# jwliao1209/DiffMusic

Hardware: AMD Instinct MI355X
Metric: denoising steps/sec (10 s clip, 200-step DPS) (higher is better)
Workload: dtype f16; 1 GPU; MusicLDM + DPS music_inpainting, 10 s @16 kHz, 200-step schedule, batch 8 per GPU (BASELINE.json configs[1]); global_batch=8, clips_per_gpu=8, lanes=1, parallelism=clip-sharded x1 (RCCL world size 1, no per-step collective), finite=True, nan_steps=0, settle_steps=10, cached_reference_transform=True, launched_by=single process

## Files before the change

diffmusic_amd/_lib.py:

```python
import ctypes as C
import os

_HERE = os.path.dirname(os.path.abspath(__file__))
LIB_PATH = os.environ.get("DMX_LIB_PATH") or os.path.join(_HERE, "lib", "libdiffmusic_hip.so")
MAX_STAGES = 8


class HifiGanConfig(C.Structure):
    _fields_ = [("model_in_dim", C.c_int), ("upsample_initial_channel", C.c_int), ("num_upsamples", C.c_int),
                ("upsample_rates", C.c_int * MAX_STAGES), ("upsample_kernel_sizes", C.c_int * MAX_STAGES),
                ("num_kernels", C.c_int), ("resblock_kernel_sizes", C.c_int * MAX_STAGES),
                ("num_dilations", C.c_int), ("resblock_dilation_sizes", C.c_int * (MAX_STAGES * MAX_STAGES)),
                ("leaky_relu_slope", C.c_float)]


class VaeConfig(C.Structure):
    _fields_ = [("latent_channels", C.c_int), ("out_channels", C.c_int), ("num_blocks", C.c_int),
                ("block_out_channels", C.c_int * MAX_STAGES), ("layers_per_block", C.c_int),
                ("norm_num_groups", C.c_int), ("eps", C.c_float)]


class UNetConfig(C.Structure):
    _fields_ = [("in_channels", C.c_int), ("out_channels", C.c_int), ("num_blocks", C.c_int),
                ("block_out_channels", C.c_int * MAX_STAGES), ("layers_per_block", C.c_int),
# ... 69 lines not shown
    "dmx_unet_workspace_bytes": (C.c_size_t, [C.c_void_p, C.c_int, C.c_int, C.c_int]),
    "dmx_unet_fwd": (C.c_int, [C.c_void_p, C.c_void_p, C.c_void_p, C.c_void_p, C.c_void_p, C.c_int, C.c_int, C.c_int,
                               C.c_void_p, C.c_size_t, C.c_void_p]),
    "dmx_unet_fwd_ctx": (C.c_int, [C.c_void_p] * 5 + [C.c_int, C.c_void_p, C.c_int, C.c_void_p, C.c_void_p, C.c_int, C.c_int, C.c_int,
                                   C.c_void_p, C.c_size_t, C.c_void_p]),
    "dmx_unet_workspace_bytes_ctx": (C.c_size_t, [C.c_void_p, C.c_int, C.c_int, C.c_int, C.c_int, C.c_int]),
    "dmx_htsat_create": (C.c_void_p, [C.POINTER(HtsatConfig)]),
    "dmx_htsat_feature_dims": (C.c_int, [C.c_void_p, C.POINTER(C.c_int), C.POINTER(C.c_int)]),
    "dmx_htsat_workspace_bytes": (C.c_size_t, [C.c_void_p, C.c_int, C.c_int]),
    "dmx_htsat_fwd": (C.c_int, [C.c_void_p, C.c_void_p, C.c_int, C.c_int, C.c_void_p, C.c_int, C.c_void_p, C.c_size_t, C.c_void_p]),
    "dmx_htsat_bwd": (C.c_int, [C.c_void_p, C.c_void_p, C.c_void_p, C.c_void_p, C.c_void_p]),
    "dmx_htsat_tape_raw": (C.c_size_t, [C.c_void_p, C.c_int, C.c_int, C.c_int, C.c_void_p, C.c_size_t, C.c_void_p]),
    "dmx_gram_fwd": (C.c_int, [C.c_void_p, C.c_void_p, C.c_int, C.c_int, C.c_int, C.c_void_p]),
    "dmx_gram_bwd": (C.c_int, [C.c_void_p, C.c_void_p, C.c_void_p, C.c_int, C.c_int, C.c_int, C.c_void_p]),
    "dmx_gemm_raw": (C.c_int, [C.c_void_p, C.c_size_t, C.c_void_p]),
    "dmx_prof_begin": (None, []),
    "dmx_prof_end": (C.c_int, [C.POINTER(C.c_double), C.POINTER(C.c_double)]),
    "dmx_flash_attn_raw": (C.c_int, [C.c_void_p, C.c_void_p, C.c_void_p, C.c_void_p, C.c_void_p] + [C.c_int] * 6 + [C.c_float, C.c_void_p]),
    "dmx_flash_attn_ld_raw": (C.c_int, [C.c_void_p] * 5 + [C.c_int] * 8 + [C.c_float, C.POINTER(C.c_int), C.c_void_p]),
    "dmx_softmax_raw": (C.c_int, [C.c_void_p] * 3 + [C.c_longlong, C.c_int, C.c_longlong, C.c_longlong, C.c_int, C.c_void_p]),
    "dmx_softmax_act_raw": (C.c_int, [C.c_void_p] * 3 + [C.c_longlong, C.c_int, C.c_longlong, C.c_int, C.c_void_p]),
    "dmx_transpose_raw": (C.c_int, [C.c_void_p, C.c_void_p, C.c_int, C.c_int, C.c_longlong, C.c_longlong, C.c_int, C.c_int] + [C.c_longlong] * 4
                          + [C.c_void_p]),
    "dmx_rowdot_raw": (C.c_int, [C.c_void_p] * 3 + [C.c_longlong, C.c_int, C.c_longlong, C.c_longlong, C.c_void_p]),
    "dmx_layernorm_raw": (C.c_int, [C.c_void_p] * 4 + [C.c_int, C.c_int, C.c_float, C.c_void_p]),
    "dmx_geglu_raw": (C.c_int, [C.c_void_p, C.c_void_p, C.c_longlong, C.c_int, C.c_void_p]),
    "dmx_gemm_splitk_workspace": (C.c_int, [C.c_void_p, C.c_size_t]),
    "dmx_conv_pair_raw": (C.c_int, [C.c_void_p, C.c_void_p, C.c_size_t, C.c_void_p]),
    "dmx_conv_pair_group_raw": (C.c_int, [C.c_int, C.c_void_p, C.c_void_p, C.c_size_t, C.c_void_p]),
    "dmx_conv_pair_dead_raw": (C.c_int, [C.c_void_p, C.c_void_p, C.c_size_t, C.POINTER(C.c_int), C.POINTER(C.c_int), C.POINTER(C.c_int), C.c_void_p]),
# ... 150 lines not shown
```

diffmusic_amd/csrc/capi.hip:

```cpp
#include "conv_pair.h"
#include "models.h"

#define M_IMPL(m) ((m) ? (m)->impl : nullptr)
#define ST(s) ((hipStream_t)(s))

extern "C" {

int dmx_abi_version(void) { return DMX_ABI_VERSION; }
int dmx_act_dtype(void) { return DMX_ACT_DTYPE; }

dmx_model* dmx_hifigan_create(const dmx_hifigan_config* cfg) {
  if (!cfg || cfg->num_upsamples > DMX_MAX_STAGES || cfg->num_kernels > DMX_MAX_STAGES || cfg->num_dilations > DMX_MAX_STAGES) {
    dmx_set_error("bad hifigan config");
    return nullptr;
  }
  return new dmx_model{dmx_make_hifigan(cfg)};
}
dmx_model* dmx_vae_decoder_create(const dmx_vae_config* cfg) {
  if (!cfg || cfg->num_blocks > DMX_MAX_STAGES) { dmx_set_error("bad vae config"); return nullptr; }
  Model* m = dmx_make_vae(cfg);
  return m ? new dmx_model{m} : nullptr;
}
dmx_model* dmx_unet_create(const dmx_unet_config* cfg) {
  if (!cfg || cfg->num_blocks > DMX_MAX_STAGES) { dmx_set_error("bad unet config"); return nullptr; }
// ... 143 lines not shown
                 void* ws, size_t ws_bytes, void* stream) {
  int rc = check(m, DMX_MODEL_UNET);
  if (rc) return rc;
  if (!ws) { dmx_set_error("null workspace"); return DMX_ERR_WORKSPACE; }
  return dmx_unet_fwd_impl(m->impl, x, t, class_labels, eps, batch, h, w, ws, ws_bytes, ST(stream), nullptr, 0, nullptr, 0, nullptr);
}
int dmx_unet_fwd_ctx(dmx_model* m, const float* x, const float* t, const float* class_labels, const float* ctx0, int n0,
                     const float* ctx1, int n1, const float* bias1, float* eps, int batch, int h, int w, void* ws, size_t ws_bytes,
                     void* stream) {
  int rc = check(m, DMX_MODEL_UNET);
  if (rc) return rc;
  if (!ws) { dmx_set_error("null workspace"); return DMX_ERR_WORKSPACE; }
  return dmx_unet_fwd_impl(m->impl, x, t, class_labels, eps, batch, h, w, ws, ws_bytes, ST(stream), ctx0, n0, ctx1, n1, bias1);
}

static thread_local int g_raw_gn_rows = 0;
int dmx_gemm_raw(const void* desc, size_t desc_bytes, void* stream) {
  if (desc_bytes != sizeof(GemmDesc)) { dmx_set_error("GemmDesc size mismatch: %zu vs %zu", desc_bytes, sizeof(GemmDesc)); return DMX_ERR_SHAPE; }
  return dmx_gemm_launch(*reinterpret_cast<const GemmDesc*>(desc), ST(stream), &g_raw_gn_rows);
}
int dmx_gemm_last_tile_rows_raw(void) { return g_raw_gn_rows; }

int dmx_conv_pair_raw(const void* desc_a, const void* desc_b, size_t desc_bytes, void* stream) {
  if (desc_bytes != sizeof(GemmDesc)) { dmx_set_error("GemmDesc size mismatch: %zu vs %zu", desc_bytes, sizeof(GemmDesc)); return DMX_ERR_SHAPE; }
  const GemmDesc* a = reinterpret_cast<const GemmDesc*>(desc_a);
  const GemmDesc& b = *reinterpret_cast<const GemmDesc*>(desc_b);
  if (!dmx_conv_pair_eligible(a, b)) { dmx_set_error("shape not handled by the fused convolution-pair kernel"); return DMX_ERR_SHAPE; }
  return dmx_conv_pair_launch(a, b, ST(stream));
}

// ... 149 lines not shown
```

diffmusic_amd/csrc/dmx_common.h:

```cpp
#pragma once
#include <hip/hip_runtime.h>
#include <stdint.h>
#include <stddef.h>

typedef uint16_t act_t;

#define DMX_OK 0
#define DMX_ERR_SHAPE (-1)
#define DMX_ERR_WORKSPACE (-2)
#define DMX_ERR_PARAM (-3)
#define DMX_ERR_STATE (-4)
#define DMX_ERR_LAUNCH (-5)

typedef __attribute__((ext_vector_type(4))) float f32x4;
#ifdef DMX_BF16
typedef __bf16 native16_t;
typedef __attribute__((ext_vector_type(8))) __bf16 frag8_t;
#define DMX_MFMA16(a, b, c) __builtin_amdgcn_mfma_f32_16x16x32_bf16(a, b, c, 0, 0, 0)
#define DMX_ACT_DTYPE 0
#else
typedef _Float16 native16_t;
typedef __attribute__((ext_vector_type(8))) _Float16 frag8_t;
#define DMX_MFMA16(a, b, c) __builtin_amdgcn_mfma_f32_16x16x32_f16(a, b, c, 0, 0, 0)
#define DMX_ACT_DTYPE 1
// ... 108 lines not shown
  const act_t* gnb_x;
  const float* gnb_scale;
  const float* gnb_shift;
  int gnb_ldx, gnb_silu;
  const float* gnb_stats;
  int gnb_cpg;
};

int dmx_gemm_launch(const GemmDesc& d, hipStream_t stream, int* gn_rows = nullptr);
void dmx_gemm_set_splitk_workspace(float* ws, size_t bytes);
void dmx_gemm_release_splitk_workspace(const float* ws);
int dmx_gemm_launch_ln(int cfg, const GemmDesc& d, hipStream_t stream);
int dmx_gemm_launch_rowstats(int cfg, const GemmDesc& d, hipStream_t stream);
int dmx_gemm_launch_gnstats(int cfg, const GemmDesc& d, hipStream_t stream, int* gn_rows);
bool dmx_prof_is_active();
```

diffmusic_amd/csrc/gemm_conv.hip:

```cpp
#include "gemm_tile.h"

namespace {
template <int BM, int BN, int WM, int WN, int NSTAGE>
int launch_glds(const GemmDesc& d, hipStream_t stream) {
  if (d.flags & EPI_SOFTBWD) {
    if constexpr (BM == 256 && BN == 256) return launch_glds_t<BM, BN, WM, WN, NSTAGE, 2>(d, stream);
    else return DMX_ERR_SHAPE;
  }
  if (d.flags & EPI_GEGLU) return launch_glds_t<BM, BN, WM, WN, NSTAGE, 3>(d, stream);
  return (d.flags & (EPI_MASKBITS | EPI_BITS2)) ? launch_glds_t<BM, BN, WM, WN, NSTAGE, 1>(d, stream)
                                                : launch_glds_t<BM, BN, WM, WN, NSTAGE, 0>(d, stream);
}

template <int BM, int BN, int WM, int WN>
int launch_cfg(const GemmDesc& d, hipStream_t stream) {
  if (d.flags & EPI_SOFTBWD) return DMX_ERR_SHAPE;
  if (d.flags & EPI_GEGLU) {
    if constexpr ((BN / WN) % 32 == 0) return launch_cfg_t<BM, BN, WM, WN, 3>(d, stream);
    else return DMX_ERR_SHAPE;
  }
  return (d.flags & (EPI_MASKBITS | EPI_BITS2)) ? launch_cfg_t<BM, BN, WM, WN, 1>(d, stream) : launch_cfg_t<BM, BN, WM, WN, 0>(d, stream);
}

}

#include <vector>
// ... 5 lines not shown
int g_last_cfg = 0;
bool g_prof = false;
std::vector<ProfRec> g_prof_recs;
struct TileEntry { int M, N, K, Z, cfg; };
static const TileEntry g_tile_table[] = {
#include "tile_table.inc"
    {0, 0, 0, 0, 0}};

bool glds_ok(const GemmDesc& d) {
  const long long imgs = d.Hq * d.Wq > 0 ? (d.M + (long long)d.Hq * d.Wq - 1) / ((long long)d.Hq * d.Wq) : 1;
  const long long in_elems = (d.Hi > 1 || d.ntaps > 1 ? imgs * d.Hi * d.Wi : (long long)d.M) * d.lda;
  static const bool strided_ok = getenv("DMX_NO_GLDS_STRIDED") == nullptr;
  return in_elems < (1ll << 29) && (long long)d.M * d.lda < (1ll << 29) && ((long long)d.N + 512) * d.ldw < (1ll << 29) &&
         (d.sy == 1 || strided_ok);
}
int launch_by_cfg(int cfg, const GemmDesc& d, hipStream_t stream, int* gn_rows = nullptr) {
  g_last_cfg = cfg;
  if (d.flags & EPI_LNFOLD) return dmx_gemm_launch_ln(cfg, d, stream);
  if (d.flags & EPI_ROWSTATS) return dmx_gemm_launch_rowstats(cfg, d, stream);
  if (d.flags & (EPI_GNSTATS | EPI_GNBWD)) return dmx_gemm_launch_gnstats(cfg, d, stream, gn_rows);
  switch (cfg) {
    case 1: return launch_glds<256, 256, 2, 4, 2>(d, stream);
    case 2: return launch_glds<256, 128, 4, 2, 3>(d, stream);
    case 7: return launch_glds<320, 256, 2, 4, 2>(d, stream);
    case 8: return launch_glds<192, 256, 2, 4, 2>(d, stream);
    case 9: return launch_glds<320, 128, 4, 2, 2>(d, stream);
    case 10: return launch_glds<192, 128, 4, 2, 3>(d, stream);
    case 11: return launch_glds<128, 128, 2, 2, 2>(d, stream);
    case 12: return launch_glds<64, 64, 2, 2, 4>(d, stream);
    case 13: return launch_glds<128, 64, 2, 2, 3>(d, stream);
    case 14: return launch_glds<64, 128, 2, 2, 3>(d, stream);
    case 15: return launch_glds<64, 64, 2, 2, 8>(d, stream);
    case 16: return launch_glds<64, 128, 2, 2, 6>(d, stream);
    case 17: return launch_glds<128, 64, 2, 2, 6>(d, stream);
    case 18: return launch_glds<128, 128, 2, 2, 4>(d, stream);
    case 19: return launch_glds<512, 128, 4, 2, 2>(d, stream);
    case 3: return launch_cfg<128, 128, 2, 2>(d, stream);
    case 4: return launch_cfg<128, 64, 2, 2>(d, stream);
    case 5: return launch_cfg<128, 32, 4, 1>(d, stream);
    default: return launch_cfg<64, 64, 2, 2>(d, stream);
  }
}
int launch_dispatch(const GemmDesc& d, hipStream_t stream, int* gn_rows) {
  const bool gl = glds_ok(d);
  if (d.flags & EPI_SOFTBWD) return gl ? launch_by_cfg(1, d, stream, gn_rows) : DMX_ERR_SHAPE;
  if (d.tile_cfg >= 1 && d.tile_cfg <= 19 && ((d.tile_cfg > 2 && d.tile_cfg < 7) || gl)) return launch_by_cfg(d.tile_cfg, d, stream, gn_rows);
  {
    static int ovN[8], ovC[8], nov = -1;
    if (nov < 0) {
      nov = 0;
      if (const char* e = getenv("DMX_CFG_OVERRIDE")) {
        while (*e && nov < 8) {
          int n = 0, c = 0;
          if (sscanf(e, "%d:%d", &n, &c) == 2) { ovN[nov] = n; ovC[nov] = c; ++nov; }
          while (*e && *e != ',') ++e;
          if (*e == ',') ++e;
        }
      }
    }
    if (gl && d.M >= 40000)
      for (int i = 0; i < nov; ++i) if (ovN[i] == d.N) return launch_by_cfg(ovC[i], d, stream, gn_rows);
  }
  for (const TileEntry* e = g_tile_table; e->cfg; ++e)
    if (e->M == d.M && e->N == d.N && e->K == d.K && e->Z == d.Z) {
      const int c = e->cfg % 100;
      if ((c > 2 && c < 7) || gl) return launch_by_cfg(c, d, stream, gn_rows);
    }
  if (gl && d.M >= 2048 && d.N % 128 == 0) {
    auto cost = [&](int bm, int bn, int slots, double eff) {
      const double blocks = (double)cdiv(d.M, bm) * cdiv(d.N, bn) * d.Z;
      const double rounds = ceil(blocks / slots);
      return rounds * (bm / 128.0) * (bn / 128.0) * (slots / 256.0) / eff;
    };
    struct Cand { int cfg, bm, bn, slots; double eff; };
    static const Cand cands[] = {{1, 256, 256, 256, 0.95}, {7, 320, 256, 256, 0.93}, {8, 192, 256, 256, 0.88},
                                 {2, 256, 128, 256, 0.70}, {9, 320, 128, 256, 0.70}, {10, 192, 128, 256, 0.66},
                                 {19, 512, 128, 256, 0.75},
                                 {3, 128, 128, 512, 0.66}};
    int best = 0;
    double bc = 1e30;
    for (const Cand& c : cands) {
      if (c.bn == 256 && d.N % 256) continue;
      const double v = cost(c.bm, c.bn, c.slots, c.eff);
      if (v < bc) { bc = v; best = c.cfg; }
    }
    if (best && best != 3) return launch_by_cfg(best, d, stream, gn_rows);
  }
  if (d.N > 32 && (long long)cdiv(d.M, 128) * cdiv(d.N, 128) * d.Z < 200) {
    if (gl && d.K >= 512 && d.Z == 1) return launch_by_cfg(d.N % 128 == 0 && d.M >= 4000 ? 14 : 12, d, stream, gn_rows);
    return launch_by_cfg(6, d, stream, gn_rows);
  }
  if (d.N > 64) return launch_by_cfg(3, d, stream, gn_rows);
  if (d.N > 32) return launch_by_cfg(4, d, stream, gn_rows);
  return launch_by_cfg(5, d, stream, gn_rows);
}
}

bool dmx_prof_is_active() { return g_prof; }

extern "C" void dmx_prof_begin(void) {
// ... 14 lines not shown
  if (flops) *flops = g_dma_fl;
  if (bytes) *bytes = g_dma_by;
  return g_dma_n;
}
extern "C" int dmx_prof_end(double* total_ms, double* total_flops) {
  g_prof = false;
  g_dma_ms = g_dma_fl = g_dma_by = 0.0; g_dma_n = 0;
  (void)hipDeviceSynchronize();
  double ms = 0.0, fl = 0.0;
  FILE* csv = getenv("DMX_PROF_CSV") ? fopen(getenv("DMX_PROF_CSV"), "w") : nullptr;
  if (csv) fprintf(csv, "M,N,K,Z,taps,flags,cfg,ms,tflops\n");
  for (auto& r : g_prof_recs) {
    float t = 0.f;
    if (hipEventElapsedTime(&t, r.a, r.b) == hipSuccess) ms += t;
    if (csv) fprintf(csv, "%d,%d,%d,%d,%d,%d,%d,%.4f,%.1f\n", r.M, r.N, r.K, r.Z, r.taps, r.flags, r.cfg, t, t > 0 ? r.flops / t / 1e9 : 0.0);
    const bool dma = r.cfg == 1 || r.cfg == 2 || (r.cfg >= 7 && r.cfg <= 10) || r.cfg == 19;
    if (dma) { g_dma_ms += t; g_dma_fl += r.flops; g_dma_by += r.bytes; ++g_dma_n; }
    fl += r.flops;
    (void)hipEventDestroy(r.a); (void)hipEventDestroy(r.b);
  }
  if (csv) fclose(csv);
  const int n = (int)g_prof_recs.size();
  g_prof_recs.clear();
  if (total_ms) *total_ms = ms;
  if (total_flops) *total_flops = fl;
  return n;
}

namespace {
float* g_splitk_ws = nullptr;
size_t g_splitk_bytes = 0;
// ... 184 lines not shown
```

diffmusic_amd/csrc/gemm_tile.h:

```cpp
#pragma once
#include "dmx_common.h"
#include <type_traits>
#include <cstdlib>

#include "gemm_epilogue.h"
#include "conv_pair.h"

namespace {

constexpr int BK = 64;
constexpr int DMX_DEF_BIG = 0;

template <int BM, int BN, int NT>
__device__ __forceinline__ void ln_prologue(const GemmDesc& p, int m0, int n0, float2* s_ln, float* s_cs) {
  constexpr int TPR = NT / BM >= 4 ? 4 : (NT / BM >= 2 ? 2 : 1);
  const int tid = threadIdx.x, ns = p.nslots;
  const int r = tid / TPR, sub = tid - r * TPR;
  const float inv_c = 1.f / (float)p.K;
  if (r < BM) {
    const int m = m0 + r;
    const bool row_ok = m < p.M;
    const float2* rs = reinterpret_cast<const float2*>(p.rowstats_in) + (long long)(row_ok ? m : 0) * ns;
    float si = 0.f, qi = 0.f;
    for (int t0 = 0; t0 < ns; t0 += TPR * 8) {
// ... 194 lines not shown
    constexpr int EPI_WAVE_BYTES = EPI_CH * (FN * 32 + 16) + EPI_CH * 12;
    static_assert(EPI_WAVE_BYTES * WM * WN <= 2 * (BM + BN) * 128, "epilogue staging does not fit the stage buffers");
    gemm_epilogue_lds<FM, FN, EM>(p, acc, m0t + wm * TM, tn * BN + wn * TN, lane, coff, HqWq, smem + wave * EPI_WAVE_BYTES, mlim);
  }
}

constexpr unsigned OOB = 0x80000000u;

#ifdef DMX_GEMM_STAMPS
__device__ unsigned long long g_gemm_stamps[8192 * 6];
#define DMX_GSTAMP(i) do { gstamp_v[i] = wall_clock64(); } while (0)
#else
#define DMX_GSTAMP(i) do { } while (0)
#endif

template <int BM, int BN, int WM, int WN, int NSTAGE, int EM, bool LNF = false>
__device__ __forceinline__ void glds_tile(const GemmDesc& p, char* smem, const int m0, const int tn, const int mlim) {
  constexpr int NW = WM * WN;
  constexpr int TM = BM / WM, TN = BN / WN;
  constexpr int FM = TM / 16, FN = TN / 16;
  constexpr int A_ISS = BM / 8 / NW, B_ISS = BN / 8 / NW;
  constexpr int A_BYTES = BM * 128, B_BYTES = BN * 128, STAGE = A_BYTES + B_BYTES;
  static_assert(A_ISS >= 1 && B_ISS >= 1, "tile too small");

  constexpr int PER = A_ISS + B_ISS;
  constexpr int KEEP = (NSTAGE - 2) * PER;

  const int tid = threadIdx.x;
  const int wave = __builtin_amdgcn_readfirstlane(tid >> 6), lane = tid & 63;
#ifdef DMX_GEMM_STAMPS
  unsigned long long gstamp_v[5] = {0, 0, 0, 0, 0};
#endif
  DMX_GSTAMP(0);
  const int z = blockIdx.y;
  const int zo = z / p.Zi, zi = z - zo * p.Zi;
  const act_t* Ab = p.A + zo * p.sAo + zi * p.sAi;
  const act_t* Wb = p.W + zo * p.sWo + zi * p.sWi;
  const int nsplit = p.ksplit > 1 ? p.ksplit : 1, sp = blockIdx.z;
  const long long coff = zo * p.sCo + zi * p.sCi + (nsplit > 1 ? (long long)sp * p.M * p.N : 0ll);
  const __amdgpu_buffer_rsrc_t rsA = __builtin_amdgcn_make_buffer_rsrc(const_cast<act_t*>(Ab), 0, OOB, 0x00020000);
  const __amdgpu_buffer_rsrc_t rsW = __builtin_amdgcn_make_buffer_rsrc(const_cast<act_t*>(Wb), 0, (unsigned)p.N * (unsigned)p.ldw * 2u, 0x00020000);

  int tapreg = 0;
#pragma unroll
  for (int j = 0; j < DMX_MAX_TAPS; ++j)
    if (lane == j) tapreg = (int)(unsigned char)p.tdy[j] | ((int)(unsigned char)p.tdx[j] << 8);

  const int lrow = lane >> 3, cc = (lane & 7) ^ lrow;
  const int cpt = p.Ci >> 3;
  const int HqWq = p.Hq * p.Wq;
  const unsigned lda2 = (unsigned)p.lda * 2u;
  unsigned a_lin[A_ISS], a_mask2[(A_ISS + 1) / 2];
  {
    int r_iy[A_ISS], r_ix[A_ISS];
    unsigned r_mask[A_ISS];
#pragma unroll
    for (int i = 0; i < A_ISS; ++i) {
      const int m = m0 + (i * NW + wave) * 8 + lrow;
      r_mask[i] = 0u; a_lin[i] = 0u;
      r_iy[i] = -(1 << 20); r_ix[i] = 0;
      if (m < mlim) {
        int b = 0, qy = 0, qx = m;
        if (!(p.Hq == 1 && p.Wq >= p.M)) {
          b = m / HqWq; const int rem = m - b * HqWq;
          qy = rem / p.Wq; qx = rem - qy * p.Wq;
        }
        r_iy[i] = qy * p.sy; r_ix[i] = qx * p.sx;
        a_lin[i] = (unsigned)b * (unsigned)(p.Hi * p.Wi) * lda2 + (unsigned)(r_iy[i] * p.Wi + r_ix[i]) * lda2 + ((unsigned)cc << 4);
// ... 14 lines not shown
  const unsigned ldw2 = (unsigned)p.ldw * 2u;
  const unsigned w_row = (unsigned)(tn * BN + wave * 8 + lrow) * ldw2;
  const unsigned w_step = (unsigned)(NW * 8) * ldw2;

  const int kchunks = p.K >> 3;
  const bool tap_inner = (p.Ci & 63) == 0 || p.ntaps == 1;
  const int cgroups = (p.Ci + 63) >> 6;
  const int nk_all = (p.K + BK - 1) / BK;
  const int ks_per = (nk_all + nsplit - 1) / nsplit;
  const int ks0 = sp * ks_per, ks1 = ks0 + ks_per < nk_all ? ks0 + ks_per : nk_all;
  int i_cg = ks0 / p.ntaps, i_tp = ks0 - i_cg * p.ntaps;
  bool q_kval = false;
  int q_tp = 0;
  unsigned q_adel = 0, q_wdel = 0;
  char* q_base = nullptr;
  auto issue_begin = [&](int ksl, int stage) {
    q_base = smem + stage * STAGE;
    if (tap_inner) {
      const int tp = __builtin_amdgcn_readfirstlane(i_tp), cgi = __builtin_amdgcn_readfirstlane(i_cg);
      q_kval = cgi < cgroups && ksl + ks0 < ks1 && cgi * 8 + cc < cpt;
      const int tv = __builtin_amdgcn_readlane(tapreg, tp);
      const int dy = (int)(signed char)(tv & 0xff), dx = (int)(signed char)((tv >> 8) & 0xff);
      q_tp = tp;
      q_adel = (unsigned)((dy * p.Wi + dx) * (int)lda2) + ((unsigned)cgi << 7);
      q_wdel = (unsigned)(tp * cpt + cgi * 8 + cc) << 4;
      if (++i_tp == p.ntaps) { i_tp = 0; ++i_cg; }
    } else {
      const int ks = ksl + ks0;
      const int kc = ks * 8 + cc;
      const int tap = kc / cpt;
      q_kval = kc < kchunks && ks < ks1;
      const int tv = __builtin_amdgcn_ds_bpermute((tap & (DMX_MAX_TAPS - 1)) << 2, tapreg);
      const int dy = (int)(signed char)(tv & 0xff), dx = (int)(signed char)((tv >> 8) & 0xff);
      q_tp = tap & (DMX_MAX_TAPS - 1);
      q_adel = (unsigned)((dy * p.Wi + dx) * (int)lda2) + ((unsigned)(kc - tap * cpt) << 4) - ((unsigned)cc << 4);
      q_wdel = (unsigned)kc << 4;
    }
  };
  auto issue_one = [&](auto I) {
    constexpr int i = decltype(I)::value;
    if constexpr (i < A_ISS) {
      const bool ok = q_kval && ((a_mask2[i >> 1] >> ((i & 1) * 16 + q_tp)) & 1u);
      const unsigned voff = ok ? a_lin[i] + q_adel : OOB;
      __builtin_amdgcn_raw_ptr_buffer_load_lds(rsA, (__attribute__((address_space(3))) void*)(q_base + (i * NW + wave) * 1024), 16, voff, 0, 0, 0);
    } else {
      constexpr int j = i - A_ISS;
      const unsigned voff = q_kval ? w_row + (unsigned)j * w_step + q_wdel : OOB;
      __builtin_amdgcn_raw_ptr_buffer_load_lds(rsW, (__attribute__((address_space(3))) void*)(q_base + A_BYTES + (j * NW + wave) * 1024), 16, voff, 0, 0, 0);
    }
  };
  auto issue = [&](int ksl, int stage) {
    issue_begin(ksl, stage);
    static_for<0, PER>(issue_one);
  };

  const int wm = wave / WN, wn = wave - wm * WN;
// ... 3 lines not shown
#pragma unroll
    for (int j = 0; j < FN; ++j) {
      const int n = tn * BN + wn * TN + j * 16 + lq * 4;
      const float4 bb = n < p.N ? *reinterpret_cast<const float4*>(p.bias + n) : make_float4(0.f, 0.f, 0.f, 0.f);
#pragma unroll
      for (int i = 0; i < FM; ++i) acc[i][j] = f32x4{bb.x, bb.y, bb.z, bb.w};
    }
  } else {
#pragma unroll
    for (int i = 0; i < FM; ++i)
#pragma unroll
      for (int j = 0; j < FN; ++j) acc[i][j] = f32x4{0.f, 0.f, 0.f, 0.f};
  }

  const int nk = ks1 > ks0 ? ks1 - ks0 : 0;
#pragma unroll
  for (int s = 0; s < NSTAGE - 1; ++s) issue(s, s);
  float2* s_ln = reinterpret_cast<float2*>(smem + NSTAGE * STAGE);
  float* s_cs = reinterpret_cast<float*>(smem + NSTAGE * STAGE + BM * 8);
  if constexpr (LNF) ln_prologue<BM, BN, NW * 64>(p, m0, tn * BN, s_ln, s_cs);
  asm volatile("s_waitcnt vmcnt(%0)" ::"n"(KEEP) : "memory");
  __builtin_amdgcn_s_barrier();
  DMX_GSTAMP(1);

  constexpr int NS = 2 * FM;
  constexpr int P0 = FN + 2;
  constexpr bool ROOMY = FM * FN * 4 + 4 * FM + 8 * FN + 64 <= 256;
  constexpr bool STAGGER = NW == 8 && FM >= 2 && (ROOMY || DMX_DEF_BIG > 0);
  constexpr int DEF = ROOMY ? FM : (DMX_DEF_BIG > 0 ? (DMX_DEF_BIG < FM ? DMX_DEF_BIG : FM) : 1);
  constexpr int LOWN = NS - DEF;
  static_assert(DEF <= FM && DEF >= 1, "carried steps must all be kk = 1 steps");
  frag8_t wf0[FN], wf1[FN], af[NS];
#define DMX_DSR(dst, addr, off) asm volatile("ds_read_b128 %0, %1 offset:%2" : "=v"(dst) : "v"(addr), "n"(off))
  auto kloop = [&](auto LAGT) {
    constexpr bool LAG = decltype(LAGT)::value;
    int cur = 0, nxt = NSTAGE - 1;
    auto mfma_step = [&wf0, &wf1, &af, &acc](auto ST) {
      constexpr int st = decltype(ST)::value;
      constexpr int kk = st / FM, i = st - kk * FM;
#pragma unroll
      for (int j = 0; j < FN; ++j) acc[i][j] = DMX_MFMA16(kk ? wf1[j] : wf0[j], af[st], acc[i][j]);
      __builtin_amdgcn_sched_barrier(0);
    };
    for (int ks = 0; ks < nk; ++ks) {
      const char* sa = smem + cur * STAGE + (wm * TM + lr) * 128;
      const char* sb = smem + cur * STAGE + A_BYTES + (wn * TN + lr) * 128;
      const unsigned a0 = (unsigned)(size_t)(__attribute__((address_space(3))) const char*)(sa);
      const unsigned b0 = (unsigned)(size_t)(__attribute__((address_space(3))) const char*)(sb);
      const unsigned sw0 = ((0 * 4 + lq) ^ (lr & 7)) << 4, sw1 = ((1 * 4 + lq) ^ (lr & 7)) << 4;
      const unsigned aA0 = a0 + sw0, aA1 = a0 + sw1, aB0 = b0 + sw0, aB1 = b0 + sw1;
      __builtin_amdgcn_sched_barrier(0);
      constexpr bool P0_LATE = LAG && DEF < FM;
      auto prologue_reads = [&wf0, &af, aA0, aA1, aB0]() {
        static_for<0, FN>([&wf0, aB0](auto J) { constexpr int j = decltype(J)::value; DMX_DSR(wf0[j], aB0, j * 2048); });
        DMX_DSR(af[0], aA0, 0);
        if constexpr (FM > 1) { DMX_DSR(af[1], aA0, 2048); } else { DMX_DSR(af[1], aA1, 0); }
      };
      if constexpr (!P0_LATE) prologue_reads();
      auto read_step = [&wf1, &af, aA0, aA1, aB1](auto ST) {
        constexpr int st = decltype(ST)::value;
        if constexpr (st + 2 < NS) {
          constexpr int s2 = st + 2, k2 = s2 / FM, i2 = s2 - k2 * FM;
          if constexpr (k2 == 0) { DMX_DSR(af[s2], aA0, i2 * 2048); } else { DMX_DSR(af[s2], aA1, i2 * 2048); }
        }
        if constexpr (LAG && st >= LOWN - (DEF - 2) && st < LOWN) {
// ... 43 lines not shown
        static_for<0, NS>([&](auto ST) {
          constexpr int st = decltype(ST)::value;
          read_step(ST);
          wait_step(ST);
          mfma_step(ST);
          if constexpr (st < SPREAD) {
            static_for<st * PER / SPREAD, (st + 1) * PER / SPREAD>(issue_one);
            __builtin_amdgcn_sched_barrier(0);
          }
        });
      }
      asm volatile("s_waitcnt vmcnt(%0)\n\ts_waitcnt lgkmcnt(0)" ::"n"(KEEP) : "memory");
      __builtin_amdgcn_s_barrier();
      cur = cur + 1 == NSTAGE ? 0 : cur + 1;
      nxt = nxt + 1 == NSTAGE ? 0 : nxt + 1;
    }
    if constexpr (LAG) {
      __builtin_amdgcn_sched_barrier(0);
      if (nk > 0) static_for<LOWN, NS>(mfma_step);
    }
  };
  if constexpr (STAGGER) {
    if (wave >= NW / 2) kloop(std::true_type{}); else kloop(std::false_type{});
  } else {
    kloop(std::false_type{});
  }
#undef DMX_DSR
  asm volatile("s_waitcnt vmcnt(0)" ::: "memory");
  __builtin_amdgcn_s_barrier();
  DMX_GSTAMP(2);
// ... 17 lines not shown
      asm volatile("s_getreg_b32 %0, hwreg(HW_REG_HW_ID)" : "=s"(hw));
      asm volatile("s_getreg_b32 %0, hwreg(HW_REG_XCC_ID)" : "=s"(xcc));
#pragma unroll
      for (int i = 0; i < 5; ++i) g_gemm_stamps[wg * 6 + i] = gstamp_v[i];
      g_gemm_stamps[wg * 6 + 5] = ((unsigned long long)(xcc & 0xf) << 32) | hw;
    }
  }
#endif
}

__device__ __forceinline__ int xcd_remap(int bid) {
  const int nwg = gridDim.x, q = nwg >> 3, r = nwg & 7, xcd = bid & 7, loc = bid >> 3;
  return (xcd < r ? xcd * (q + 1) : r * (q + 1) + (xcd - r) * q) + loc;
}

template <int BM, int BN, int WM, int WN, int NSTAGE, int EM, bool LNF = false>
__global__ __launch_bounds__(WM* WN * 64) void gemm_glds_kernel(const GemmDesc p) {
  extern __shared__ __attribute__((aligned(16))) char smem[];
  const int tiles_n = (p.N + BN - 1) / BN;
  const int bid = xcd_remap(blockIdx.x);
  int m0 = (bid / tiles_n) * BM, mlim = p.M;
  if constexpr (EM == 5 || EM == 6) {
    const int P = p.Hq * p.Wq;
    if (P % (BM / WM) != 0) {
      const int tpi = (P + BM - 1) / BM, tm = bid / tiles_n, b = tm / tpi;
      m0 = b * P + (tm - b * tpi) * BM;
      mlim = (b + 1) * P;
    }
  }
  glds_tile<BM, BN, WM, WN, NSTAGE, EM, LNF>(p, smem, m0, bid % tiles_n, mlim);
}

template <int BM, int BN, int WM, int WN, int NSTAGE, int EM, bool LNF = false>
int launch_glds_t(const GemmDesc& d, hipStream_t stream) {
  constexpr int NT = WM * WN * 64;
  constexpr int SMEM = NSTAGE * (BM + BN) * 128 + (LNF ? BM * 8 + BN * 8 : 0);
  static_assert(SMEM <= 160 * 1024, "tile ring exceeds the 160 KiB of LDS");
  static bool attr_set = false;
  if (!attr_set) {
    hipFuncSetAttribute(reinterpret_cast<const void*>(&gemm_glds_kernel<BM, BN, WM, WN, NSTAGE, EM, LNF>),
                        hipFuncAttributeMaxDynamicSharedMemorySize, SMEM);
    attr_set = true;
  }
  long long tiles = (long long)cdiv(d.M, BM) * cdiv(d.N, BN);
  if constexpr (EM == 5 || EM == 6) {
    const int P = d.Hq * d.Wq;
    if (P % (BM / WM) != 0) tiles = (long long)(d.M / P) * cdiv(P, BM) * cdiv(d.N, BN);
  }
  dim3 grid((unsigned)tiles, (unsigned)d.Z, (unsigned)(d.ksplit > 1 ? d.ksplit : 1));
  static const bool bias_init = getenv("DMX_NO_BIAS_INIT") == nullptr;
  if (bias_init && (d.flags & EPI_BIAS) && d.bias && !(d.flags & (EPI_MASK | EPI_MASKBITS | EPI_SOFTBWD | EPI_LNFOLD))) {
    GemmDesc q = d;
    q.flags = (q.flags & ~EPI_BIAS) | EPI_BIASINIT;
    hipLaunchKernelGGL((gemm_glds_kernel<BM, BN, WM, WN, NSTAGE, EM, LNF>), grid, dim3(NT), SMEM, stream, q);
    return hipGetLastError() == hipSuccess ? DMX_OK : DMX_ERR_LAUNCH;
  }
  hipLaunchKernelGGL((gemm_glds_kernel<BM, BN, WM, WN, NSTAGE, EM, LNF>), grid, dim3(NT), SMEM, stream, d);
  return hipGetLastError() == hipSuccess ? DMX_OK : DMX_ERR_LAUNCH;
}
template <int BM, int BN, int WM, int WN, int EM, bool LNF = false>
int launch_cfg_t(const GemmDesc& d, hipStream_t stream) {
  constexpr int NT = WM * WN * 64;
  constexpr int SMEM = 2 * (BM + BN) * 128 + DMX_MAX_TAPS * 4 + (LNF ? BM * 8 + BN * 8 : 0);
  static bool attr_set = false;
  if (!attr_set) {
    hipFuncSetAttribute(reinterpret_cast<const void*>(&gemm_kernel<BM, BN, WM, WN, EM, LNF>),
                        hipFuncAttributeMaxDynamicSharedMemorySize, SMEM);
    attr_set = true;
  }
  long long tiles = (long long)cdiv(d.M, BM) * cdiv(d.N, BN);
  if constexpr (EM == 5 || EM == 6) {
    const int P = d.Hq * d.Wq;
// ... 15 lines not shown
```

include/diffmusic_hip.h:

```cpp
#ifndef DIFFMUSIC_HIP_H
#define DIFFMUSIC_HIP_H
#include <stddef.h>
#include <stdint.h>

#ifdef __cplusplus
extern "C" {
#endif

#define DMX_ABI_VERSION 4
#define DMX_MAX_STAGES 8

typedef struct dmx_model dmx_model;

typedef struct dmx_hifigan_config {
  int model_in_dim;
  int upsample_initial_channel;
  int num_upsamples;
  int upsample_rates[DMX_MAX_STAGES];
  int upsample_kernel_sizes[DMX_MAX_STAGES];
  int num_kernels;
  int resblock_kernel_sizes[DMX_MAX_STAGES];
  int num_dilations;
  int resblock_dilation_sizes[DMX_MAX_STAGES * DMX_MAX_STAGES];
  float leaky_relu_slope;
// ... 206 lines not shown
int dmx_sched_cfg_combine(const float* eps2, float* out, long long n, float scale, void* stream);
int dmx_sched_step(int mode, const float* x, const float* eps, const float* x0, const float* g0, const float* inv_scale,
                   const float* noise, float* prev, float* x0_out, float* grad_out, int batch, int n, float alpha_t, float alpha_prev,
                   float sigma, float rate, float eps_small, int global_norm, void* stream);
int dmx_sched_step_ex(int mode, const float* x, const float* eps, const float* x0, const float* g0, const float* inv_scale,
                      const float* noise, float* prev, float* x0_out, float* grad_out, int batch, int n, float alpha_t, float alpha_prev,
                      float sigma, float rate, float eps_small, int global_norm, int prediction_type, float clip_range, void* stream);

int dmx_randn_philox(float* out, int batch, long long n, const unsigned long long* seeds_host, unsigned long long offset, void* stream);

void dmx_prof_begin(void);
int dmx_prof_end(double* total_ms, double* total_flops);
int dmx_prof_dominant(double* ms, double* flops, double* bytes);

int dmx_gemm_raw(const void* desc, size_t desc_bytes, void* stream);
int dmx_flash_attn_raw(const void* q, const void* k, const void* v, void* o, const float* colbias, int B, int Nq, int Nk, int ldv,
                       int C, int heads, float scale, void* stream);
int dmx_flash_attn_ld_raw(const void* q, const void* k, const void* v, void* o, const float* colbias, int B, int Nq, int Nk, int ldq,
                          int ldk, int ldv, int C, int heads, float scale, int* qt_out, void* stream);
int dmx_softmax_raw(const float* S, void* P, const float* colbias, long long rows, int N, long long lds, long long ldp, int rows_per_bias,
                    void* stream);
int dmx_softmax_act_raw(const void* S, void* P, const float* colbias, long long rows, int N, long long ldp, int rows_per_bias, void* stream);
int dmx_transpose_raw(const void* in, void* out, int R, int C, long long ldi, long long ldo, int Z, int Zi, long long sIo, long long sIi,
                      long long sOo, long long sOi, void* stream);
int dmx_rowdot_raw(const void* a, const void* b, float* out, long long rows, int C, long long lda, long long ldb, void* stream);
int dmx_layernorm_raw(const void* x, void* y, const float* gamma, const float* beta, int rows, int C, float eps, void* stream);
int dmx_geglu_raw(const void* x, void* y, long long rows, int I, void* stream);
int dmx_gemm_splitk_workspace(void* ws, size_t bytes);
int dmx_conv_pair_raw(const void* desc_a, const void* desc_b, size_t desc_bytes, void* stream);
int dmx_conv_pair_dead_raw(const void* desc_a, const void* desc_b, size_t desc_bytes, const int* dead, int* skipped, int* total, void* stream);
// ... 20 lines not shown
```

Baseline: 26.68 steps/s (weak scaling: one step advances a batch of 8 clips on one GPU; value = K / wall x 1 GPU(s)).

## Add slab-reuse implicit-GEMM path for 1D multi-tap convs

Adds a slab mode to the LDS-DMA GEMM kernel for 1D (Hi=1) multi-tap convolutions. Instead of reloading an A tile for every tap, it loads one 320+64-row slab per channel group, double-buffered, and indexes each tap by a row shift inside LDS. Only the weight tile flows through the stage ring. Tiles are assigned per image so the halo stays within a row. The path is chosen automatically where cfg 7 was picked and the shape and tap count qualify. This cuts global/LDS A traffic by roughly the tap count, at the cost of a different pipeline schedule and more occupancy pressure from LDS use. DMX_NO_SLAB disables it.

```diff
diff --git a/diffmusic_amd/_lib.py b/diffmusic_amd/_lib.py
--- a/diffmusic_amd/_lib.py
+++ b/diffmusic_amd/_lib.py
@@ -107,6 +107,8 @@
     "dmx_gram_fwd": (C.c_int, [C.c_void_p, C.c_void_p, C.c_int, C.c_int, C.c_int, C.c_void_p]),
     "dmx_gram_bwd": (C.c_int, [C.c_void_p, C.c_void_p, C.c_void_p, C.c_int, C.c_int, C.c_int, C.c_void_p]),
     "dmx_gemm_raw": (C.c_int, [C.c_void_p, C.c_size_t, C.c_void_p]),
+    "dmx_gemm_slab_eligible": (C.c_int, [C.c_void_p, C.c_size_t]),
+    "dmx_gemm_last_cfg_raw": (C.c_int, []),
     "dmx_prof_begin": (None, []),
     "dmx_prof_end": (C.c_int, [C.POINTER(C.c_double), C.POINTER(C.c_double)]),
     "dmx_flash_attn_raw": (C.c_int, [C.c_void_p, C.c_void_p, C.c_void_p, C.c_void_p, C.c_void_p] + [C.c_int] * 6 + [C.c_float, C.c_void_p]),
diff --git a/diffmusic_amd/csrc/capi.hip b/diffmusic_amd/csrc/capi.hip
--- a/diffmusic_amd/csrc/capi.hip
+++ b/diffmusic_amd/csrc/capi.hip
@@ -181,6 +181,11 @@
   return dmx_unet_fwd_impl(m->impl, x, t, class_labels, eps, batch, h, w, ws, ws_bytes, ST(stream), ctx0, n0, ctx1, n1, bias1);
 }
 
+int dmx_gemm_slab_eligible(const void* desc, size_t desc_bytes) {
+  if (!desc || desc_bytes != sizeof(GemmDesc)) { dmx_set_error("GemmDesc size mismatch: %zu vs %zu", desc_bytes, sizeof(GemmDesc)); return DMX_ERR_SHAPE; }
+  return dmx_gemm_slab_ok(*reinterpret_cast<const GemmDesc*>(desc)) ? 1 : 0;
+}
+int dmx_gemm_last_cfg_raw(void) { return dmx_gemm_last_cfg(); }
 static thread_local int g_raw_gn_rows = 0;
 int dmx_gemm_raw(const void* desc, size_t desc_bytes, void* stream) {
   if (desc_bytes != sizeof(GemmDesc)) { dmx_set_error("GemmDesc size mismatch: %zu vs %zu", desc_bytes, sizeof(GemmDesc)); return DMX_ERR_SHAPE; }
diff --git a/diffmusic_amd/csrc/dmx_common.h b/diffmusic_amd/csrc/dmx_common.h
--- a/diffmusic_amd/csrc/dmx_common.h
+++ b/diffmusic_amd/csrc/dmx_common.h
@@ -146,3 +146,5 @@
 int dmx_gemm_launch_rowstats(int cfg, const GemmDesc& d, hipStream_t stream);
 int dmx_gemm_launch_gnstats(int cfg, const GemmDesc& d, hipStream_t stream, int* gn_rows);
 bool dmx_prof_is_active();
+bool dmx_gemm_slab_ok(const GemmDesc& d);
+int dmx_gemm_last_cfg();
diff --git a/diffmusic_amd/csrc/gemm_conv.hip b/diffmusic_amd/csrc/gemm_conv.hip
--- a/diffmusic_amd/csrc/gemm_conv.hip
+++ b/diffmusic_amd/csrc/gemm_conv.hip
@@ -10,6 +10,12 @@
   if (d.flags & EPI_GEGLU) return launch_glds_t<BM, BN, WM, WN, NSTAGE, 3>(d, stream);
   return (d.flags & (EPI_MASKBITS | EPI_BITS2)) ? launch_glds_t<BM, BN, WM, WN, NSTAGE, 1>(d, stream)
                                                 : launch_glds_t<BM, BN, WM, WN, NSTAGE, 0>(d, stream);
+}
+
+template <int S>
+int launch_slab(const GemmDesc& d, hipStream_t stream) {
+  return (d.flags & (EPI_MASKBITS | EPI_BITS2)) ? launch_glds_t<320, 256, 2, 4, 2, 1, false, S>(d, stream)
+                                                : launch_glds_t<320, 256, 2, 4, 2, 0, false, S>(d, stream);
 }
 
 template <int BM, int BN, int WM, int WN>
@@ -45,8 +51,40 @@
   return in_elems < (1ll << 29) && (long long)d.M * d.lda < (1ll << 29) && ((long long)d.N + 512) * d.ldw < (1ll << 29) &&
          (d.sy == 1 || strided_ok);
 }
+}
+
+bool dmx_gemm_slab_ok(const GemmDesc& d) {
+  if (d.Hi != 1 || d.Hq != 1 || d.sx != 1 || d.ntaps < 2 || d.ntaps > DMX_MAX_TAPS || (d.Ci & 63) || d.Ci <= 0 || d.N <= 0 || (d.N & 255)) return false;
+  if (d.Wq <= 0 || d.M % d.Wq != 0 || d.ksplit > 1) return false;
+  int lo = 127, hi = -128;
+  for (int t = 0; t < d.ntaps; ++t) {
+    if (d.tdy[t] != 0) return false;
+    lo = d.tdx[t] < lo ? d.tdx[t] : lo;
+    hi = d.tdx[t] > hi ? d.tdx[t] : hi;
+  }
+  if (hi - lo > SLAB_HALO) return false;
+  if (d.flags & (EPI_F32OUT | EPI_SOFTBWD | EPI_GEGLU | EPI_LNFOLD | EPI_ROWSTATS | EPI_GNSTATS | EPI_GNBWD)) return false;
+  if ((d.ldc | d.ldr | d.ldx | d.ldc2) & 7) return false;
+  return glds_ok(d);
+}
+int dmx_gemm_last_cfg() { return g_last_cfg; }
+
+namespace {
+inline int slab_cfg(int ntaps) { return ntaps >= 6 ? 21 : (ntaps >= 3 ? 20 : 22); }
+int slab_adopt(const GemmDesc& d) {
+  static const bool no_slab = getenv("DMX_NO_SLAB") != nullptr;
+  if (no_slab || !(d.N == 256 || d.N == 512) || !(d.ntaps == 3 || d.ntaps == 7 || d.ntaps == 11) || d.Z != 1 || !dmx_gemm_slab_ok(d)) return 7;
+  const long long flat = (long long)cdiv(d.M, 320) * (d.N / 256), per_image = (long long)(d.M / d.Wq) * cdiv(d.Wq, 320) * (d.N / 256);
+  return (per_image + 255) / 256 <= (flat + 255) / 256 ? slab_cfg(d.ntaps) : 7;
+}
+
 int launch_by_cfg(int cfg, const GemmDesc& d, hipStream_t stream, int* gn_rows = nullptr) {
   g_last_cfg = cfg;
+  if (cfg >= 20 && cfg <= 22) {
+    const int S = cfg == 20 ? 2 : (cfg == 21 ? 1 : 3);
+    if (!dmx_gemm_slab_ok(d) || d.ntaps * S < 6) return DMX_ERR_SHAPE;
+    return S == 2 ? launch_slab<2>(d, stream) : (S == 1 ? launch_slab<1>(d, stream) : launch_slab<3>(d, stream));
+  }
   if (d.flags & EPI_LNFOLD) return dmx_gemm_launch_ln(cfg, d, stream);
   if (d.flags & EPI_ROWSTATS) return dmx_gemm_launch_rowstats(cfg, d, stream);
   if (d.flags & (EPI_GNSTATS | EPI_GNBWD)) return dmx_gemm_launch_gnstats(cfg, d, stream, gn_rows);
@@ -75,7 +113,7 @@
 int launch_dispatch(const GemmDesc& d, hipStream_t stream, int* gn_rows) {
   const bool gl = glds_ok(d);
   if (d.flags & EPI_SOFTBWD) return gl ? launch_by_cfg(1, d, stream, gn_rows) : DMX_ERR_SHAPE;
-  if (d.tile_cfg >= 1 && d.tile_cfg <= 19 && ((d.tile_cfg > 2 && d.tile_cfg < 7) || gl)) return launch_by_cfg(d.tile_cfg, d, stream, gn_rows);
+  if (d.tile_cfg >= 1 && d.tile_cfg <= 22 && ((d.tile_cfg > 2 && d.tile_cfg < 7) || gl)) return launch_by_cfg(d.tile_cfg, d, stream, gn_rows);
   {
     static int ovN[8], ovC[8], nov = -1;
     if (nov < 0) {
@@ -94,7 +132,8 @@
   }
   for (const TileEntry* e = g_tile_table; e->cfg; ++e)
     if (e->M == d.M && e->N == d.N && e->K == d.K && e->Z == d.Z) {
-      const int c = e->cfg % 100;
+      int c = e->cfg % 100;
+      if (c == 7) c = slab_adopt(d);
       if ((c > 2 && c < 7) || gl) return launch_by_cfg(c, d, stream, gn_rows);
     }
   if (gl && d.M >= 2048 && d.N % 128 == 0) {
@@ -115,6 +154,7 @@
       const double v = cost(c.bm, c.bn, c.slots, c.eff);
       if (v < bc) { bc = v; best = c.cfg; }
     }
+    if (best == 7) best = slab_adopt(d);
     if (best && best != 3) return launch_by_cfg(best, d, stream, gn_rows);
   }
   if (d.N > 32 && (long long)cdiv(d.M, 128) * cdiv(d.N, 128) * d.Z < 200) {
@@ -159,7 +199,7 @@
     float t = 0.f;
     if (hipEventElapsedTime(&t, r.a, r.b) == hipSuccess) ms += t;
     if (csv) fprintf(csv, "%d,%d,%d,%d,%d,%d,%d,%.4f,%.1f\n", r.M, r.N, r.K, r.Z, r.taps, r.flags, r.cfg, t, t > 0 ? r.flops / t / 1e9 : 0.0);
-    const bool dma = r.cfg == 1 || r.cfg == 2 || (r.cfg >= 7 && r.cfg <= 10) || r.cfg == 19;
+    const bool dma = r.cfg == 1 || r.cfg == 2 || (r.cfg >= 7 && r.cfg <= 10) || (r.cfg >= 19 && r.cfg <= 22);
     if (dma) { g_dma_ms += t; g_dma_fl += r.flops; g_dma_by += r.bytes; ++g_dma_n; }
     fl += r.flops;
     (void)hipEventDestroy(r.a); (void)hipEventDestroy(r.b);
diff --git a/diffmusic_amd/csrc/gemm_tile.h b/diffmusic_amd/csrc/gemm_tile.h
--- a/diffmusic_amd/csrc/gemm_tile.h
+++ b/diffmusic_amd/csrc/gemm_tile.h
@@ -232,7 +232,9 @@
 #define DMX_GSTAMP(i) do { } while (0)
 #endif
 
-template <int BM, int BN, int WM, int WN, int NSTAGE, int EM, bool LNF = false>
+constexpr int SLAB_HALO = 64;
+
+template <int BM, int BN, int WM, int WN, int NSTAGE, int EM, bool LNF = false, int SLAB = 0>
 __device__ __forceinline__ void glds_tile(const GemmDesc& p, char* smem, const int m0, const int tn, const int mlim) {
   constexpr int NW = WM * WN;
   constexpr int TM = BM / WM, TN = BN / WN;
@@ -240,8 +242,11 @@
   constexpr int A_ISS = BM / 8 / NW, B_ISS = BN / 8 / NW;
   constexpr int A_BYTES = BM * 128, B_BYTES = BN * 128, STAGE = A_BYTES + B_BYTES;
   static_assert(A_ISS >= 1 && B_ISS >= 1, "tile too small");
-
-  constexpr int PER = A_ISS + B_ISS;
+  constexpr int SLAB_BYTES = (BM + SLAB_HALO) * 128, SLAB_ISS = (BM + SLAB_HALO) / 8 / NW;
+  constexpr int W_OFF = SLAB > 0 ? 2 * SLAB_BYTES : A_BYTES, W_STAGE = SLAB > 0 ? B_BYTES : STAGE;
+  static_assert(SLAB == 0 || (NSTAGE == 2 && !LNF && (BM + SLAB_HALO) % (8 * NW) == 0 && TM % 8 == 0), "slab loop: two stages, whole pieces per wave");
+
+  constexpr int PER = SLAB > 0 ? B_ISS + SLAB : A_ISS + B_ISS;
   constexpr int KEEP = (NSTAGE - 2) * PER;
 
   const int tid = threadIdx.x;
@@ -269,7 +274,18 @@
   const int HqWq = p.Hq * p.Wq;
   const unsigned lda2 = (unsigned)p.lda * 2u;
   unsigned a_lin[A_ISS], a_mask2[(A_ISS + 1) / 2];
-  {
+  int s_ix0 = 0, s_lo = 0;
+  unsigned s_lin0 = 0u;
+  if constexpr (SLAB > 0) {
+    s_lo = 127;
+    for (int t = 0; t < p.ntaps; ++t) {
+      const int dx = (int)(signed char)((__builtin_amdgcn_readlane(tapreg, t) >> 8) & 0xff);
+      s_lo = dx < s_lo ? dx : s_lo;
+    }
+    const int b = m0 / HqWq;
+    s_ix0 = m0 - b * HqWq + s_lo + wave * 8 + lrow;
+    s_lin0 = ((unsigned)b * (unsigned)p.Wi + (unsigned)s_ix0) * lda2 + ((unsigned)cc << 4);
+  } else {
     int r_iy[A_ISS], r_ix[A_ISS];
     unsigned r_mask[A_ISS];
 #pragma unroll
@@ -314,7 +330,30 @@
   int q_tp = 0;
   unsigned q_adel = 0, q_wdel = 0;
   char* q_base = nullptr;
+  int c_tp = 0, c_cg = 0;
+  int q_pi0 = 0;
+  bool q_sval = false;
+  unsigned q_sdel = 0;
+  char* q_sbase = nullptr;
+  auto slab_piece = [&](int pi, char* base, unsigned del) {
+    const int ix = s_ix0 + pi * (NW * 8);
+    const unsigned voff = (unsigned)ix < (unsigned)p.Wi ? s_lin0 + (unsigned)(pi * (NW * 8)) * lda2 + del : OOB;
+    __builtin_amdgcn_raw_ptr_buffer_load_lds(rsA, (__attribute__((address_space(3))) void*)(base + (pi * NW + wave) * 1024), 16, voff, 0, 0, 0);
+  };
   auto issue_begin = [&](int ksl, int stage) {
+    if constexpr (SLAB > 0) {
+      const int tp = __builtin_amdgcn_readfirstlane(i_tp), cgi = __builtin_amdgcn_readfirstlane(i_cg);
+      q_base = smem + W_OFF + stage * W_STAGE;
+      q_kval = cgi < cgroups;
+      q_wdel = (unsigned)(tp * cpt + cgi * 8 + cc) << 4;
+      if (++i_tp == p.ntaps) { i_tp = 0; ++i_cg; }
+      const int ctp = __builtin_amdgcn_readfirstlane(c_tp), ccg = __builtin_amdgcn_readfirstlane(c_cg);
+      q_pi0 = ctp * SLAB;
+      q_sval = ccg + 1 < cgroups;
+      q_sdel = (unsigned)(ccg + 1) << 7;
+      q_sbase = smem + ((ccg + 1) & 1) * SLAB_BYTES;
+      return;
+    }
     q_base = smem + stage * STAGE;
     if (tap_inner) {
       const int tp = __builtin_amdgcn_readfirstlane(i_tp), cgi = __builtin_amdgcn_readfirstlane(i_cg);
@@ -339,7 +378,13 @@
   };
   auto issue_one = [&](auto I) {
     constexpr int i = decltype(I)::value;
-    if constexpr (i < A_ISS) {
+    if constexpr (SLAB > 0 && i >= B_ISS) {
+      const int pi = q_pi0 + (i - B_ISS);
+      if (pi < SLAB_ISS && q_sval) slab_piece(pi, q_sbase, q_sdel);
+    } else if constexpr (SLAB > 0) {
+      const unsigned voff = q_kval ? w_row + (unsigned)i * w_step + q_wdel : OOB;
+      __builtin_amdgcn_raw_ptr_buffer_load_lds(rsW, (__attribute__((address_space(3))) void*)(q_base + (i * NW + wave) * 1024), 16, voff, 0, 0, 0);
+    } else if constexpr (i < A_ISS) {
       const bool ok = q_kval && ((a_mask2[i >> 1] >> ((i & 1) * 16 + q_tp)) & 1u);
       const unsigned voff = ok ? a_lin[i] + q_adel : OOB;
       __builtin_amdgcn_raw_ptr_buffer_load_lds(rsA, (__attribute__((address_space(3))) void*)(q_base + (i * NW + wave) * 1024), 16, voff, 0, 0, 0);
@@ -373,8 +418,14 @@
   }
 
   const int nk = ks1 > ks0 ? ks1 - ks0 : 0;
-#pragma unroll
-  for (int s = 0; s < NSTAGE - 1; ++s) issue(s, s);
+  if constexpr (SLAB > 0) {
+    static_for<0, SLAB_ISS>([&](auto PI) { slab_piece(decltype(PI)::value, smem, 0u); });
+    issue_begin(0, 0);
+    static_for<0, B_ISS>(issue_one);
+  } else {
+#pragma unroll
+    for (int s = 0; s < NSTAGE - 1; ++s) issue(s, s);
+  }
   float2* s_ln = reinterpret_cast<float2*>(smem + NSTAGE * STAGE);
   float* s_cs = reinterpret_cast<float*>(smem + NSTAGE * STAGE + BM * 8);
   if constexpr (LNF) ln_prologue<BM, BN, NW * 64>(p, m0, tn * BN, s_ln, s_cs);
@@ -389,6 +440,7 @@
   constexpr int DEF = ROOMY ? FM : (DMX_DEF_BIG > 0 ? (DMX_DEF_BIG < FM ? DMX_DEF_BIG : FM) : 1);
   constexpr int LOWN = NS - DEF;
   static_assert(DEF <= FM && DEF >= 1, "carried steps must all be kk = 1 steps");
+  static_assert(SLAB == 0 || !STAGGER, "the slab loop exists for the unstaggered 320-row tile");
   frag8_t wf0[FN], wf1[FN], af[NS];
 #define DMX_DSR(dst, addr, off) asm volatile("ds_read_b128 %0, %1 offset:%2" : "=v"(dst) : "v"(addr), "n"(off))
   auto kloop = [&](auto LAGT) {
@@ -402,12 +454,25 @@
       __builtin_amdgcn_sched_barrier(0);
     };
     for (int ks = 0; ks < nk; ++ks) {
-      const char* sa = smem + cur * STAGE + (wm * TM + lr) * 128;
-      const char* sb = smem + cur * STAGE + A_BYTES + (wn * TN + lr) * 128;
-      const unsigned a0 = (unsigned)(size_t)(__attribute__((address_space(3))) const char*)(sa);
-      const unsigned b0 = (unsigned)(size_t)(__attribute__((address_space(3))) const char*)(sb);
-      const unsigned sw0 = ((0 * 4 + lq) ^ (lr & 7)) << 4, sw1 = ((1 * 4 + lq) ^ (lr & 7)) << 4;
-      const unsigned aA0 = a0 + sw0, aA1 = a0 + sw1, aB0 = b0 + sw0, aB1 = b0 + sw1;
+      unsigned aA0, aA1, aB0, aB1;
+      if constexpr (SLAB > 0) {
+        const int tp = __builtin_amdgcn_readfirstlane(c_tp), cg = __builtin_amdgcn_readfirstlane(c_cg);
+        const int dx = (int)(signed char)((__builtin_amdgcn_readlane(tapreg, tp) >> 8) & 0xff);
+        const int row = wm * TM + lr + (dx - s_lo);
+        const char* sa = smem + (cg & 1) * SLAB_BYTES + row * 128;
+        const char* sb = smem + W_OFF + cur * W_STAGE + (wn * TN + lr) * 128;
+        const unsigned a0 = (unsigned)(size_t)(__attribute__((address_space(3))) const char*)(sa);
+        const unsigned b0 = (unsigned)(size_t)(__attribute__((address_space(3))) const char*)(sb);
+        aA0 = a0 + (((0 * 4 + lq) ^ (row & 7)) << 4); aA1 = a0 + (((1 * 4 + lq) ^ (row & 7)) << 4);
+        aB0 = b0 + (((0 * 4 + lq) ^ (lr & 7)) << 4); aB1 = b0 + (((1 * 4 + lq) ^ (lr & 7)) << 4);
+      } else {
+        const char* sa = smem + cur * STAGE + (wm * TM + lr) * 128;
+        const char* sb = smem + cur * STAGE + A_BYTES + (wn * TN + lr) * 128;
+        const unsigned a0 = (unsigned)(size_t)(__attribute__((address_space(3))) const char*)(sa);
+        const unsigned b0 = (unsigned)(size_t)(__attribute__((address_space(3))) const char*)(sb);
+        const unsigned sw0 = ((0 * 4 + lq) ^ (lr & 7)) << 4, sw1 = ((1 * 4 + lq) ^ (lr & 7)) << 4;
+        aA0 = a0 + sw0; aA1 = a0 + sw1; aB0 = b0 + sw0; aB1 = b0 + sw1;
+      }
       __builtin_amdgcn_sched_barrier(0);
       constexpr bool P0_LATE = LAG && DEF < FM;
       auto prologue_reads = [&wf0, &af, aA0, aA1, aB0]() {
@@ -481,6 +546,7 @@
       __builtin_amdgcn_s_barrier();
       cur = cur + 1 == NSTAGE ? 0 : cur + 1;
       nxt = nxt + 1 == NSTAGE ? 0 : nxt + 1;
+      if constexpr (SLAB > 0) { if (++c_tp == p.ntaps) { c_tp = 0; ++c_cg; } }
     }
     if constexpr (LAG) {
       __builtin_amdgcn_sched_barrier(0);
@@ -528,7 +594,7 @@
   return (xcd < r ? xcd * (q + 1) : r * (q + 1) + (xcd - r) * q) + loc;
 }
 
-template <int BM, int BN, int WM, int WN, int NSTAGE, int EM, bool LNF = false>
+template <int BM, int BN, int WM, int WN, int NSTAGE, int EM, bool LNF = false, int SLAB = 0>
 __global__ __launch_bounds__(WM* WN * 64) void gemm_glds_kernel(const GemmDesc p) {
   extern __shared__ __attribute__((aligned(16))) char smem[];
   const int tiles_n = (p.N + BN - 1) / BN;
@@ -542,17 +608,22 @@
       mlim = (b + 1) * P;
     }
   }
-  glds_tile<BM, BN, WM, WN, NSTAGE, EM, LNF>(p, smem, m0, bid % tiles_n, mlim);
-}
-
-template <int BM, int BN, int WM, int WN, int NSTAGE, int EM, bool LNF = false>
+  if constexpr (SLAB > 0) {
+    const int P = p.Wq, tpi = (P + BM - 1) / BM, tm = bid / tiles_n, b = tm / tpi;
+    m0 = b * P + (tm - b * tpi) * BM;
+    mlim = (b + 1) * P;
+  }
+  glds_tile<BM, BN, WM, WN, NSTAGE, EM, LNF, SLAB>(p, smem, m0, bid % tiles_n, mlim);
+}
+
+template <int BM, int BN, int WM, int WN, int NSTAGE, int EM, bool LNF = false, int SLAB = 0>
 int launch_glds_t(const GemmDesc& d, hipStream_t stream) {
   constexpr int NT = WM * WN * 64;
-  constexpr int SMEM = NSTAGE * (BM + BN) * 128 + (LNF ? BM * 8 + BN * 8 : 0);
+  constexpr int SMEM = SLAB > 0 ? 2 * (BM + SLAB_HALO + BN) * 128 : NSTAGE * (BM + BN) * 128 + (LNF ? BM * 8 + BN * 8 : 0);
   static_assert(SMEM <= 160 * 1024, "tile ring exceeds the 160 KiB of LDS");
   static bool attr_set = false;
   if (!attr_set) {
-    hipFuncSetAttribute(reinterpret_cast<const void*>(&gemm_glds_kernel<BM, BN, WM, WN, NSTAGE, EM, LNF>),
+    hipFuncSetAttribute(reinterpret_cast<const void*>(&gemm_glds_kernel<BM, BN, WM, WN, NSTAGE, EM, LNF, SLAB>),
                         hipFuncAttributeMaxDynamicSharedMemorySize, SMEM);
     attr_set = true;
   }
@@ -561,15 +632,16 @@
     const int P = d.Hq * d.Wq;
     if (P % (BM / WM) != 0) tiles = (long long)(d.M / P) * cdiv(P, BM) * cdiv(d.N, BN);
   }
+  if constexpr (SLAB > 0) tiles = (long long)(d.M / d.Wq) * cdiv(d.Wq, BM) * cdiv(d.N, BN);
   dim3 grid((unsigned)tiles, (unsigned)d.Z, (unsigned)(d.ksplit > 1 ? d.ksplit : 1));
   static const bool bias_init = getenv("DMX_NO_BIAS_INIT") == nullptr;
   if (bias_init && (d.flags & EPI_BIAS) && d.bias && !(d.flags & (EPI_MASK | EPI_MASKBITS | EPI_SOFTBWD | EPI_LNFOLD))) {
     GemmDesc q = d;
     q.flags = (q.flags & ~EPI_BIAS) | EPI_BIASINIT;
-    hipLaunchKernelGGL((gemm_glds_kernel<BM, BN, WM, WN, NSTAGE, EM, LNF>), grid, dim3(NT), SMEM, stream, q);
+    hipLaunchKernelGGL((gemm_glds_kernel<BM, BN, WM, WN, NSTAGE, EM, LNF, SLAB>), grid, dim3(NT), SMEM, stream, q);
     return hipGetLastError() == hipSuccess ? DMX_OK : DMX_ERR_LAUNCH;
   }
-  hipLaunchKernelGGL((gemm_glds_kernel<BM, BN, WM, WN, NSTAGE, EM, LNF>), grid, dim3(NT), SMEM, stream, d);
+  hipLaunchKernelGGL((gemm_glds_kernel<BM, BN, WM, WN, NSTAGE, EM, LNF, SLAB>), grid, dim3(NT), SMEM, stream, d);
   return hipGetLastError() == hipSuccess ? DMX_OK : DMX_ERR_LAUNCH;
 }
 template <int BM, int BN, int WM, int WN, int EM, bool LNF = false>
diff --git a/include/diffmusic_hip.h b/include/diffmusic_hip.h
--- a/include/diffmusic_hip.h
+++ b/include/diffmusic_hip.h
@@ -244,6 +244,8 @@
 int dmx_prof_dominant(double* ms, double* flops, double* bytes);
 
 int dmx_gemm_raw(const void* desc, size_t desc_bytes, void* stream);
+int dmx_gemm_slab_eligible(const void* desc, size_t desc_bytes);
+int dmx_gemm_last_cfg_raw(void);
 int dmx_flash_attn_raw(const void* q, const void* k, const void* v, void* o, const float* colbias, int B, int Nq, int Nk, int ldv,
                        int C, int heads, float scale, void* stream);
 int dmx_flash_attn_ld_raw(const void* q, const void* k, const void* v, void* o, const float* colbias, int B, int Nq, int Nk, int ldq,
```

After: 27.12 steps/s (weak scaling: one step advances a batch of 8 clips on one GPU; value = K / wall x 1 GPU(s)), median of 6. 1.7% higher.
